# AIR-DISCOVER/TOIST

Measured on AMD Instinct MI355X. Metric: train images/sec/node (640x640, bs=8/GPU) + matcher index bit-match, higher is better.
Workload: dtype bf16; 1 GPU; configs[1]: ResNet-101 + RoBERTa-base + 6+6 transformer, 100 queries, batch 8/GPU 640x640, 16-token captions, detection loss (labels+boxes+cardinality+contrastive_align, 5 aux layers), dropout 0.1, clip 0.1 + AdamW + EMA (fused HIP tail); random-init weights; every step a different batch (4 resident batches, 0..10 targets per image) through fixed-address inputs; global_batch=8, parallelism=dp1, launch=hipGraph replay, decoder=2 XCD-resident launches (toist_xdec_fwd / toist_xdec_bwd, one image per XCD)

## Files before the change

include/toist_hip.h:

```cpp
#ifndef TOIST_HIP_H
#define TOIST_HIP_H

#include <stddef.h>
#include <stdint.h>

#ifdef __cplusplus
extern "C" {
#endif

#define TOIST_OK 0
#define TOIST_EINVAL (-1)
#define TOIST_EHIP (-2)

#define TOIST_ABI_VERSION 1

#if defined(__GNUC__)
#define TOIST_API __attribute__((visibility("default")))
#else
#define TOIST_API
#endif

TOIST_API int toist_version(void);
TOIST_API int toist_last_error(char* buf, size_t cap);

// ... 339 lines not shown
TOIST_API int toist_attn_small_fwd(const void* q, int ldq, const void* kmat, int ldk, const void* v, int ldv, const uint8_t* key_pad, int B, int H, int S,
                         int dh, float scale, float drop_p, uint64_t seed, const uint64_t* seed_dev, void* ctx, int ldo, float* stats,
                         const float* bq, const float* bk, const float* bv, void* stream);
TOIST_API int toist_attn_small_bwd(const void* q, int ldq, const void* kmat, int ldk, const void* v, int ldv, const uint8_t* key_pad, int B, int H, int S,
                         int dh, float scale, float drop_p, uint64_t seed, const uint64_t* seed_dev, const float* stats, const void* dctx,
                         int lddo, void* dq, int lddq, void* dk, int lddk, void* dv, int lddv, const float* bq, const float* bk,
                         const float* bv, void* stream);

TOIST_API int toist_conv3x3_small(int dgrad, const void* src, const void* w, const float* shift, const void* res, void* out, int n_img, int H, int W,
                        int c_src, int c_out, int w_co, int w_ci, void* stream);

TOIST_API int toist_wgrad3x3_small_blocks(void);
TOIST_API int toist_wgrad3x3_small(const void* dy, const void* x, float* ws, int n_img, int H, int W, int c_in, int c_out, void* stream);

TOIST_API int toist_lsap(const float* cost, const int64_t* offset, const int32_t* rows, const int32_t* cols, int ld ,
               int n, int max_rows, int max_cols,
               int64_t max_cells , const int64_t* out_off, int64_t* row_idx, int64_t* col_idx, int32_t* status, void* stream);

#define TOIST_GEMM_DEFER_REDUCE 2
#define TOIST_GEMM_SPLIT_EPILOGUE 4
#define TOIST_GEMM_COLSUM_SLICES 32768
TOIST_API int toist_gemm_pick_tile(const toist_gemm* desc);
typedef struct toist_reduce_desc {
    const float* ws;
    float* out;
    const float* rscale;
    int32_t splits, M, N, ldc;
    float alpha;
    int32_t accumulate;
} toist_reduce_desc;
TOIST_API int toist_gemm_effective_split(const toist_gemm* desc);
TOIST_API int toist_splitk_reduce_batch(const toist_reduce_desc* descs, int n, void* stream);

TOIST_API int toist_opt_chunk_elems(void);
TOIST_API int toist_opt_sqnorm(const toist_opt_tensor* table, const int64_t* grads, const int32_t* chunks, int n_chunks, float* partial, void* stream);
TOIST_API int toist_opt_finish_norm(const float* partial, int n_chunks, float max_norm, float beta1, float beta2, toist_opt_state* state, void* stream);
TOIST_API int toist_opt_finish_norm_guarded(const float* partial, int n_chunks, float max_norm, float beta1, float beta2, toist_opt_state* state,
                        const int32_t* const* veto_i32, int n_veto_i32, const float* const* veto_f32, int n_veto_f32, void* stream);
TOIST_API int toist_opt_adamw_ema(const toist_opt_tensor* table, const int64_t* grads, const int32_t* chunks, int n_chunks,
                        const toist_opt_group* groups, const toist_opt_state* state, float beta1, float beta2, float eps,
                        float ema_decay, void* stream);
TOIST_API int toist_opt_adamw_ema_blocks(const toist_opt_tensor* table, const int64_t* grads, const int32_t* chunks, int n_chunks,
                               const toist_opt_group* groups, const toist_opt_state* state, float beta1, float beta2, float eps,
                               float ema_decay, int max_blocks, void* stream);

TOIST_API int toist_mask_resize_pack(const float* src, int n, int h0, int w0, int max_h, int max_w, int crop_h, int crop_w, int h, int w,
                           float threshold, uint64_t* bits, void* stream);
TOIST_API int toist_mask_resize_pack_batch(const float* src, int batch, int queries, int h0, int w0, int max_h, int max_w, const int64_t* table,
                                 int cap_h, int cap_w, long long capacity_words, float threshold, uint64_t* bits, void* stream);
TOIST_API int toist_mask_pack(const uint8_t* dense, int n, int h, int w, uint64_t* bits, void* stream);
TOIST_API int toist_mask_unpack(const uint64_t* bits, int n, int h, int w, uint8_t* dense, void* stream);
TOIST_API int toist_mask_area(const uint64_t* bits, int n, int h, int w, uint32_t* area, void* stream);
TOIST_API int toist_mask_iou(const uint64_t* dt, int n_dt, const uint64_t* gt, int n_gt, const uint8_t* iscrowd, const uint32_t* area_dt,
                   const uint32_t* area_gt, int h, int w, double* iou, void* stream);
TOIST_API int toist_mask_rle_count(const uint64_t* bits, int n, int h, int w, int32_t* column_transitions, void* stream);
TOIST_API int toist_mask_rle_emit(const uint64_t* bits, int n, int h, int w, const int64_t* column_offset, uint32_t* positions, void* stream);
TOIST_API int toist_mask_rle_counts(const uint32_t* positions, const int64_t* first_position, const int64_t* first_run, int n, int h, int w,
                          uint32_t* counts, void* stream);

TOIST_API int toist_postprocess(const void* pred_logits, int logits_bf16, const void* pred_boxes, int boxes_bf16, const void* pred_isfinal, int isfinal_bf16,
                      const int64_t* orig_sizes, int B, int Q, int C, float* scores, float* boxes, float* scores_refexp, void* stream);

TOIST_API int toist_coco_match(const double* iou, const int64_t* iou_offset, const double* dt_area, const int64_t* dt_offset, const double* gt_area,
                     const uint8_t* gt_ignore, const uint8_t* gt_crowd, const int64_t* gt_offset, int n_images, const double* area_ranges,
                     int n_ranges, const double* iou_thresholds, int n_thresholds, int32_t* dt_match, uint8_t* dt_ignore,
                     uint8_t* gt_range_ignore, uint8_t* gt_taken, void* stream);
// ... 14 lines not shown
```

toist_amd/backbone.py:

```python
import os
from collections import OrderedDict

import torch
from torch import nn

from .knobs import knob
from . import engine, functions
from . import kernels as k
from . import ops
from .misc import NestedTensor
from .position_encoding import build_position_encoding

BF16 = torch.bfloat16
FUSED_STEM = knob("TOIST_FUSED_STEM", True)


_BN_EPOCH = [0]


class FrozenBatchNorm2d(nn.Module):

    def __init__(self, n):
        super().__init__()
        self.register_buffer("weight", torch.ones(n))
# ... 125 lines not shown
    def _program(self, levels, first=1, last=4, stem=True):
        body = self.body
        bn_cache = {}

        def bn(name):
            if name not in bn_cache:
                bn_cache[name] = body.get_submodule(name).scale_shift()
            return bn_cache[name]

        def prog(tape, ps, images):
            x = images.data
            if stem:
                N, C, H, W = x.shape
                s0, t0 = bn("bn1")
                w1 = engine.krsc(ps["conv1.weight"].w)
                if FUSED_STEM and tuple(w1.shape) == (64, 7, 7, 8) and x.dtype == torch.float32:
                    CH, CW = (H - 1) // 2 + 1, (W - 1) // 2 + 1
                    pooled = torch.empty(N, (CH - 1) // 2 + 1, (CW - 1) // 2 + 1, 64, dtype=BF16, device=x.device)
                    k.stem_fwd(x.contiguous(), w1, t0, pooled)
                else:
                    xin = torch.empty(N, H, W, 8, dtype=BF16, device=x.device)
                    k.pack_image(x.contiguous(), xin)
                    y = ops.conv2d(xin, w1, stride=2, pad=3, shift=t0, act=k.ACT_RELU, cin_real=C)
                    OH, OW = (y.shape[1] + 2 - 3) // 2 + 1, (y.shape[2] + 2 - 3) // 2 + 1
                    pooled = torch.empty(N, OH, OW, 64, dtype=BF16, device=x.device)
                    k.maxpool3x3s2(y, pooled)
                    del y
                cur = engine.Var(pooled, needs_grad=False)
            else:
                cur = images
            outs = []
            for li in range(first, last + 1):
                layer = getattr(body, f"layer{li}")
                for bi, blk in enumerate(layer):
                    pre = f"layer{li}.{bi}."
                    Wd = {"conv1": ps[pre + "conv1.weight"], "conv2": ps[pre + "conv2.weight"], "conv3": ps[pre + "conv3.weight"]}
                    bnd = {"bn1": bn(pre + "bn1"), "bn2": bn(pre + "bn2"), "bn3": bn(pre + "bn3")}
                    has_down = blk.downsample is not None
                    if has_down:
                        Wd["down"] = ps[pre + "downsample.0.weight"]
                        bnd["down"] = bn(pre + "downsample.1")
                    train = Wd["conv1"].g is not None
                    nxt = engine.bottleneck(tape, cur, Wd, bnd, blk.stride, has_down, train)
                    nxt.needs_grad = train
                    cur = nxt
                if li in levels:
                    outs.append(cur)
            return outs, None

        return prog

    @staticmethod
    def _with_output_masks(prog, premasked):
        def wrapped(tape, ps, img):
            outs, extra = prog(tape, ps, img)
            finals = []
            for oi, o in enumerate(outs):
                f = engine.Var(o.data, needs_grad=o.needs_grad)

                def bwd(o=o, f=f, oi=oi):
                    g = f.take_grad()
                    if g is None or not o.needs_grad:
                        return
                    gm = g if oi in premasked else torch.where(o.data > 0, g, torch.zeros_like(g))
                    engine.accumulate(o, gm)

                tape.record(bwd)
                finals.append(f)
            return finals, extra
        return wrapped

    STAGES = ((1, 2, True), (3, 3, False), (4, 4, False))

    def forward_native(self, images, levels=(4,), premasked=(), stage_cuts=None):
        if stage_cuts is not None and tuple(levels) == (4,):
            return self._forward_staged(images, premasked, stage_cuts)
        named = engine.named_cache(self, "body", lambda: OrderedDict(self.body.named_parameters()))
        wrapped = self._with_output_masks(self._program(levels), premasked)
        return functions.run_program(wrapped, named, [images], cache=self._cache, training=self.training, transforms=self._transforms(),
                                     group_wgrads=True, store_once=lambda n, t: t.dim() == 4)

    def _forward_staged(self, images, premasked, stage_cuts):
        tr_all = self._transforms()
        caches = self.__dict__.setdefault("_stage_caches", [{} for _ in self.STAGES])
        x = images
        for si, (first, last, stem) in enumerate(self.STAGES):
            def build(first=first, last=last, stem=stem):
                keep = tuple(f"layer{li}." for li in range(first, last + 1)) + (("conv1.",) if stem else ())
                return OrderedDict((n, p) for n, p in self.body.named_parameters() if n.startswith(keep))
            named = engine.named_cache(self, f"body.stage{si}", build)
            tr = {n: f for n, f in tr_all.items() if n in named}
            is_last = si == len(self.STAGES) - 1
            prog = self._program((last,), first, last, stem)
            wrapped = self._with_output_masks(prog, premasked if is_last else (0,))
            (y,) = functions.run_program(wrapped, named, [x], cache=caches[si], training=self.training, transforms=tr, group_wgrads=True,
                                         store_once=lambda n, t: t.dim() == 4)
            if not is_last and y.requires_grad:
                leaf = y.detach().requires_grad_(True)
                stage_cuts.append((f"backbone.layer{last}", y, leaf))
                y = leaf
            x = y
        return (x,)

    def forward(self, tensor_list: NestedTensor):
        levels = (1, 2, 3, 4) if self.return_interm_layers else (4,)
        feats = self.forward_native(tensor_list.tensors, levels)
        out = OrderedDict()
        names = [str(i) for i in range(len(levels))] if self.return_interm_layers else ["0"]
        for name, f in zip(names, feats):
            x = f.permute(0, 3, 1, 2).float()
            mask = nearest_mask(tensor_list.mask, x.shape[-2:])
            out[name] = NestedTensor(x, mask)
        return out


_NEAREST_IDX = {}


# ... 43 lines not shown
```

toist_amd/csrc/gemm.hip:

```cpp
#include <cstdlib>
#include <type_traits>

#include "common.h"
#include "gemm_route.h"

namespace toist {


__device__ __forceinline__ float gelu_f(float v) { return 0.5f * v * (1.f + erff(v * 0.70710678118654752f)); }
__device__ __forceinline__ float gelu_grad_f(float a) {
    return 0.5f * (1.f + erff(a * 0.70710678118654752f)) + a * 0.3989422804014327f * __expf(-0.5f * a * a);
}

template <int N, typename F>
__device__ __forceinline__ void static_for(F&& f) {
    if constexpr (N > 0) {
        static_for<N - 1>(f);
        f(std::integral_constant<int, N - 1>{});
    }
}

struct EpiRow {
    long long crow;
    long long rrow;
// ... 2330 lines not shown
#undef TOIST_PANEL2
#undef TOIST_PANEL2_ONE
    return TOIST_OK;
}

#ifndef GEMM_UNIT
template <int NS>
static int launch_gemm128_ring(const toist_gemm& d, hipStream_t st) {
    static std::atomic<unsigned long long> done{0};
    constexpr int LDS = NS * G8_STAGE_BYTES;
    if (!lds_attr_once_flag(done, [] {
            return hipFuncSetAttribute((const void*)gemm128_kernel<TOIST_A_ROWK, TOIST_B_ROWK, NS>, hipFuncAttributeMaxDynamicSharedMemorySize, LDS) == hipSuccess &&
                   hipFuncSetAttribute((const void*)gemm128_kernel<TOIST_A_ROWK, TOIST_B_KROW, NS>, hipFuncAttributeMaxDynamicSharedMemorySize, LDS) == hipSuccess &&
                   hipFuncSetAttribute((const void*)gemm128_kernel<TOIST_A_CONV, TOIST_B_ROWK, NS>, hipFuncAttributeMaxDynamicSharedMemorySize, LDS) == hipSuccess &&
                   hipFuncSetAttribute((const void*)gemm128_kernel<TOIST_A_CONVT, TOIST_B_KROW, NS>, hipFuncAttributeMaxDynamicSharedMemorySize, LDS) == hipSuccess;
        })) {
        set_last_error("toist_gemm_bf16: cannot enable %d bytes of LDS for the 128x128 kernel", LDS);
        return TOIST_EHIP;
    }
    const int tiles = ((d.M + G8_BM - 1) / G8_BM) * ((d.N + G8_BN - 1) / G8_BN);
    dim3 grid((tiles + 7) & ~7, 1, 1);
    if (d.a_kind == TOIST_A_CONV) hipLaunchKernelGGL((gemm128_kernel<TOIST_A_CONV, TOIST_B_ROWK, NS>), grid, dim3(512), LDS, st, d);
    else if (d.a_kind == TOIST_A_CONVT) hipLaunchKernelGGL((gemm128_kernel<TOIST_A_CONVT, TOIST_B_KROW, NS>), grid, dim3(512), LDS, st, d);
    else if (d.b_kind == TOIST_B_KROW) hipLaunchKernelGGL((gemm128_kernel<TOIST_A_ROWK, TOIST_B_KROW, NS>), grid, dim3(512), LDS, st, d);
    else hipLaunchKernelGGL((gemm128_kernel<TOIST_A_ROWK, TOIST_B_ROWK, NS>), grid, dim3(512), LDS, st, d);
    return TOIST_OK;
}

static int launch_gemm128(const toist_gemm& d, hipStream_t st) {
    static const int ring = (int)tuning_knob("TOIST_G8_RING", 5);
    return (ring == 5 && d.K >= 5 * G8_BK) ? launch_gemm128_ring<5>(d, st) : launch_gemm128_ring<4>(d, st);
}

static int launch_gemm256w(const toist_gemm& d, hipStream_t st) {
    static std::atomic<unsigned long long> done{0};
    if (!lds_attr_once_flag(done, [] {
            return hipFuncSetAttribute((const void*)gemm256w_kernel<TOIST_B_KROW>, hipFuncAttributeMaxDynamicSharedMemorySize, G9_LDS) == hipSuccess &&
                   hipFuncSetAttribute((const void*)gemm256w_kernel<TOIST_B_CONVX>, hipFuncAttributeMaxDynamicSharedMemorySize, G9_LDS) == hipSuccess;
        })) {
        set_last_error("toist_gemm_bf16: cannot enable %d bytes of LDS for the 256x128 weight-gradient kernel", G9_LDS);
        return TOIST_EHIP;
    }
    const toist_gemm& dd = d;
    const int tiles = (d.M / G9_BM) * (d.N / G9_BN);
    const int nz = dd.batch * dd.split_k;
    dim3 grid((tiles + 7) & ~7, nz, 1);
    if (nz >= 8) grid = dim3(8 * ((nz + 7) / 8) * tiles, 1, 1);
    if (d.b_kind == TOIST_B_CONVX) hipLaunchKernelGGL((gemm256w_kernel<TOIST_B_CONVX>), grid, dim3(512), G9_LDS, st, dd);
    else hipLaunchKernelGGL((gemm256w_kernel<TOIST_B_KROW>), grid, dim3(512), G9_LDS, st, dd);
    return TOIST_OK;
}

static int launch_gemm128w(const toist_gemm& d, hipStream_t st) {
    static std::atomic<unsigned long long> done{0};
    if (!lds_attr_once_flag(done, [] {
            return hipFuncSetAttribute((const void*)gemm128w_kernel<TOIST_B_KROW, 4>, hipFuncAttributeMaxDynamicSharedMemorySize, 4 * G8_STAGE_BYTES) == hipSuccess &&
                   hipFuncSetAttribute((const void*)gemm128w_kernel<TOIST_B_CONVX, 4>, hipFuncAttributeMaxDynamicSharedMemorySize, 4 * G8_STAGE_BYTES) == hipSuccess &&
                   hipFuncSetAttribute((const void*)gemm128w_kernel<TOIST_B_KROW, 5>, hipFuncAttributeMaxDynamicSharedMemorySize, 5 * G8_STAGE_BYTES) == hipSuccess &&
                   hipFuncSetAttribute((const void*)gemm128w_kernel<TOIST_B_CONVX, 5>, hipFuncAttributeMaxDynamicSharedMemorySize, 5 * G8_STAGE_BYTES) == hipSuccess;
        })) {
        set_last_error("toist_gemm_bf16: cannot enable %d bytes of LDS for the 128x128 weight-gradient kernel", 5 * G8_STAGE_BYTES);
        return TOIST_EHIP;
    }
    const int tiles = ((d.M + G8_BM - 1) / G8_BM) * ((d.N + G8_BN - 1) / G8_BN);
    const toist_gemm& dd = d;
    const int nz = dd.batch * dd.split_k;
// ... 328 lines not shown
    const gemm_verdict ok = gemm_check(d);
    if (ok.code != TOIST_OK) { set_last_error("%s", ok.msg); return ok.code; }
    const gemm_plan r = gemm_route(d);
    if (r.code != TOIST_OK) { set_last_error("%s", r.msg); return r.code; }
    d.batch = r.batch, d.batch_inner = r.batch_inner, d.split_k = r.split;
    hipStream_t st = (hipStream_t)stream;
    const char* what = "toist_gemm_bf16";
    int rc;
    switch (r.family) {
        case GEMM_128: rc = launch_gemm128(d, st); what = "toist_gemm_bf16(gemm128)"; break;
        case GEMM_CONV3: rc = launch_conv3(d, st); what = "toist_gemm_bf16(conv3)"; break;
        case GEMM_PANEL: rc = r.ring == 1 ? launch_panel(d, st) : launch_panel2(d, r.ring, st); what = "toist_gemm_bf16(panel)"; break;
        case GEMM_128W: rc = launch_gemm128w(d, st); break;
        case GEMM_256W: rc = launch_gemm256w(d, st); break;
        default:
            rc = r.tile == 65 ? launch_tiles_b(r.tile, d, r.ring, st)
               : (r.tile == 130 || r.tile == 134) ? launch_tiles_c(r.tile, d, r.ring, st) : launch_tiles_a(r.tile, d, r.ring, st);
            break;
    }
    if (rc != TOIST_OK) return rc;
    rc = check_launch(what);
    if (rc != TOIST_OK || r.post == GEMM_POST_NONE || r.post == GEMM_POST_DEFERRED) return rc;
    if (r.post == GEMM_POST_EPILOGUE) {
        const long long chunks = (long long)d.M * ((d.N + 7) / 8);
        hipLaunchKernelGGL(splitk_epilogue_kernel, dim3((unsigned)((chunks + 255) / 256)), dim3(256), 0, st, d);
        return check_launch("toist_gemm_bf16(splitk epilogue)");
    }
    const long long total4 = ((long long)d.M * d.N) / 4;
    int grid = (int)((total4 + 255) / 256 > 2048 ? 2048 : (total4 + 255) / 256);
    hipLaunchKernelGGL(splitk_reduce_kernel, dim3(grid), dim3(256), 0, st, (const float*)d.workspace, d.split_k, d.M, d.N, d.epi.alpha,
                       d.epi.rscale, d.epi.accumulate, (float*)d.c, d.ldc);
    return check_launch("toist_gemm_bf16(splitk reduce)");
}
#endif
```

toist_amd/csrc/gemm_route.cpp:

```cpp
#include "gemm_route.h"

#include <cstddef>
#include <cstdio>

#include "tuning.h"

namespace toist {

static bool aligned16(const void* p) { return (((size_t)p) & 15) == 0; }

static void normalise(toist_gemm& d) {
    if (d.batch <= 0) d.batch = 1;
    if (d.batch_inner <= 0) d.batch_inner = 1;
    if (d.split_k <= 0) d.split_k = 1;
}

#define GEMM_REQUIRE(v, cond, ...) \
    do { if ((v).code == TOIST_OK && !(cond)) { (v).code = TOIST_EINVAL; std::snprintf((v).msg, sizeof((v).msg), __VA_ARGS__); } } while (0)

gemm_verdict gemm_check(const toist_gemm& desc) {
    gemm_verdict v{};
    toist_gemm d = desc;
    GEMM_REQUIRE(v, d.M > 0 && d.N > 0 && d.K > 0, "toist_gemm_bf16: bad shape M=%d N=%d K=%d", d.M, d.N, d.K);
    normalise(d);
// ... 238 lines not shown
        GEMM_REQUIRE(r, gemm128_applies(d), "toist_gemm_bf16: the 128x128 kernel does not cover this call");
    } else if (d.tile == 131 || (d.tile == 0 && d.a_kind == TOIST_A_CONVT && conv3_applies(d))) {
        r.family = GEMM_CONV3, r.tile = 131;
        GEMM_REQUIRE(r, conv3_applies(d), "toist_gemm_bf16: the 3x3 halo kernel does not cover this call");
    } else if (code == 135 || (d.tile == 0 && panel_sized && panel_applies(d))) {
        r.family = GEMM_PANEL, r.tile = 135;
        GEMM_REQUIRE(r, panel_applies(d), "toist_gemm_bf16: the short-K panel kernel does not cover this call");
        static const int def_variant = (int)tuning_knob("TOIST_PANEL_VARIANT", 0);
        const int variant = r.ring ? r.ring : def_variant;
        r.ring = (variant == 1 || !panel2_applies(d)) ? 1 : variant == 255 ? 0 : variant;
    } else {
        r.tile = code;
        if (code == 137) GEMM_REQUIRE(r, gemm128w_applies(d), "toist_gemm_bf16: the 128x128 weight-gradient kernel does not cover this call");
        if (code == 138) GEMM_REQUIRE(r, gemm256w_applies(d), "toist_gemm_bf16: the 256x128 weight-gradient kernel does not cover this call");
        if (const int wt = wgrad_tile_replaced(d)) r.tile = wt;
        if (r.tile == 0) r.tile = auto_tile(d);
        r.family = r.tile == 137 ? GEMM_128W : r.tile == 138 ? GEMM_256W : GEMM_TILES;
    }
    r.split = clamp_split(d.split_k, d.K, r.tile);
    r.post = r.split <= 1 ? GEMM_POST_NONE : (d.flags & TOIST_GEMM_DEFER_REDUCE) ? GEMM_POST_DEFERRED
           : (d.flags & TOIST_GEMM_SPLIT_EPILOGUE) ? GEMM_POST_EPILOGUE : GEMM_POST_REDUCE;
    if (r.family == GEMM_TILES || r.family == GEMM_128W || r.family == GEMM_256W) {
        if (d.flags & TOIST_GEMM_COLSUM_SLICES)
            GEMM_REQUIRE(r, r.split > 1, "toist_gemm_bf16: TOIST_GEMM_COLSUM_SLICES with a split that clamps to 1 (see toist_gemm_effective_split)");
        if (d.b_kind == TOIST_B_KROW && d.b.kin > 0) GEMM_REQUIRE(r, (d.b.kin % 8) == 0, "toist_gemm_bf16: kin %% 8 != 0");
    }
    if (r.family == GEMM_TILES) {
        GEMM_REQUIRE(r, generic_tile(r.tile), "toist_gemm_bf16: bad tile code %d", r.tile);
        GEMM_REQUIRE(r, generic_operands(d.a_kind, d.b_kind), "toist_gemm_bf16: unsupported operand kinds a=%d b=%d", d.a_kind, d.b_kind);
    }
    return r;
}

}

extern "C" int toist_gemm_pick_tile(const toist_gemm* desc) { return desc == nullptr ? 0 : toist::gemm_route(*desc).tile; }

extern "C" int toist_gemm_effective_split(const toist_gemm* desc) {
    if (desc == nullptr) return 0;
    toist_gemm d = *desc;
    if (d.workspace == nullptr) d.workspace = (float*)16;
    return toist::gemm_route(d).split;
}
```

toist_amd/csrc/gemm_route.h:

```cpp
#pragma once
#include "../../include/toist_hip.h"

namespace toist {

constexpr int C3_BM = 128, C3_BK = 64, C3_NP = 28;
constexpr int G8_BM = 128, G8_BN = 128, G8_BK = 64;
constexpr int G9_BM = 256, G9_BN = 128, G9_NS = 6;

enum gemm_family {
    GEMM_TILES = 0,
    GEMM_CONV3,
    GEMM_PANEL,
    GEMM_128,
    GEMM_128W,
    GEMM_256W
};

enum gemm_post {
    GEMM_POST_NONE = 0,
    GEMM_POST_REDUCE,
    GEMM_POST_EPILOGUE,
    GEMM_POST_DEFERRED
};

struct gemm_verdict {
    int code;
    char msg[320];
};

struct gemm_plan : gemm_verdict {
    int family;
    int tile;
    int ring;
    int batch, batch_inner, split;
    int post;
};

gemm_verdict gemm_check(const toist_gemm& desc);
gemm_plan gemm_route(const toist_gemm& desc);
bool lean_epilogue_ok(const toist_gemm& d);

}
```

toist_amd/engine.py:

```python
import math

import weakref

import torch

from . import kernels as k
from . import ops
from .knobs import knob

BF16 = torch.bfloat16


class Var:

    __slots__ = ("data", "grad", "needs_grad", "drop", "gdrop", "plus", "raw_grad")

    def __init__(self, data, needs_grad=True):
        self.data = data
        self.grad = None
        self.needs_grad = needs_grad
        self.raw_grad = False
        self.plus = None
        self.drop = None
        self.gdrop = None
# ... 749 lines not shown

def text_attention_block(tape, x, proj, Wpacked, Wo, bo, key_pad, B, L, H):
    D = Wo.w.shape[0]
    dh = D // H
    M = B * L
    dev = x.data.device
    p = tape.drop_p
    scale = 1.0 / math.sqrt(dh)
    qkv = ops.linear(x.data, Wpacked)
    seed_p = tape.next_seed() if p > 0 else 0
    ctx = torch.empty(M, D, dtype=BF16, device=dev)
    stats = torch.empty(B * H, L, 2, dtype=torch.float32, device=dev)
    bias = [b.f32 for _, b in proj]
    k.attn_small_fwd(qkv[:, :D], qkv[:, D:2 * D], qkv[:, 2 * D:], key_pad, B, H, L, dh, scale, p, seed_p, ctx, stats, *bias)
    out, head = _out_proj(tape, ctx, Wo, bo, x, p)

    def bwd():
        dctx = head()
        if dctx is None:
            return
        dqkv = torch.empty(M, 3 * D, dtype=BF16, device=dev)
        k.attn_small_bwd(qkv[:, :D], qkv[:, D:2 * D], qkv[:, 2 * D:], key_pad, B, H, L, dh, scale, p, seed_p, stats, dctx,
                         dqkv[:, :D], dqkv[:, D:2 * D], dqkv[:, 2 * D:], *bias)
        for i, (W, b) in enumerate(proj):
            if W.g is not None:
                tape.linear_wgrad(dqkv[:, i * D:(i + 1) * D], x.data, W, b)
        if x.needs_grad:
            x.grad = ops.linear_dgrad(dqkv, Wpacked, res=x.grad)

    tape.record(bwd)
    return out


def bottleneck(tape, x, W, bn, stride, has_down, train):
    w1, w2, w3 = krsc(W["conv1"].w), krsc(W["conv2"].w), krsc(W["conv3"].w)
    s1, t1 = bn["bn1"]
    s2, t2 = bn["bn2"]
    s3, t3 = bn["bn3"]
    a1 = ops.conv2d(x.data, w1, shift=t1, act=k.ACT_RELU)
    a2 = ops.conv2d(a1, w2, stride=stride, pad=1, shift=t2, act=k.ACT_RELU)
    if has_down:
        wd = krsc(W["down"].w)
        sd, td = bn["down"]
        idn = ops.conv2d(x.data, wd, stride=stride, shift=td)
    else:
        idn = x.data
    y = ops.conv2d(a2, w3, shift=t3, res=idn, act=k.ACT_RELU)
    if has_down:
        del idn
    out = Var(y)
    if not train:
        return out
    H, Wd = x.data.shape[1], x.data.shape[2]

    def bwd():
        g3 = out.take_grad()
        if g3 is None:
            return
        tape.conv_wgrad(g3, a2, w3.shape, krsc(W["conv3"].g), s3, view=W["conv3"])
        g2 = ops.conv2d_dgrad(g3, w3, a2.shape[1:3], act=k.ACT_MASK_POS, aux=a2)
        tape.conv_wgrad(g2, a1, w2.shape, krsc(W["conv2"].g), s2, stride=stride, pad=1, view=W["conv2"])
        g1 = ops.conv2d_dgrad(g2, w2, (H, Wd), stride=stride, pad=1, act=k.ACT_MASK_POS, aux=a1)
        tape.conv_wgrad(g1, x.data, w1.shape, krsc(W["conv1"].g), s1, view=W["conv1"])
        if has_down:
            tape.conv_wgrad(g3, x.data, wd.shape, krsc(W["down"].g), sd, stride=stride, view=W["down"])
        if not x.needs_grad:
            return
        prev = x.take_grad()
        if has_down:
            if stride == 1:
                gx = ops.conv2d_dgrad(g3, wd, (H, Wd), res=prev)
            else:
                gx = prev if prev is not None else torch.zeros_like(x.data)
                ops.conv2d_dgrad(g3, wd, (H, Wd), stride=stride, out=gx, res=gx if prev is not None else None)
        else:
            gx = g3
            if prev is not None:
                k.add(prev, g3, prev)
                gx = prev
        x.grad = ops.conv2d_dgrad(g1, w1, (H, Wd), res=gx, act=k.ACT_MASK_POS, aux=x.data)

    tape.record(bwd)
    return out
```

toist_amd/kernels.py:

```python
import ctypes
import os

import torch

from . import _lib
from .folds import FOLDS, _raw_stream
from .knobs import knob
from ._lib import (A_CONV, A_CONVT, A_KROW, A_ROWK, ACT_GELU, ACT_GELU_BWD, ACT_MASK_POS, ACT_NONE, ACT_RELU,
                   ACT_SIGMOID, ACT_SIGMOID_BWD, B_CONVX, B_KROW, B_ROWK, Epilogue, Gemm, Operand)

__all__ = [
    "A_ROWK", "A_KROW", "A_CONV", "A_CONVT", "B_ROWK", "B_KROW", "B_CONVX", "ACT_NONE", "ACT_RELU", "ACT_GELU",
    "ACT_SIGMOID", "ACT_MASK_POS", "ACT_GELU_BWD", "ACT_SIGMOID_BWD", "ConvGeom", "operand", "gemm", "matcher",
    "layernorm_fwd", "layernorm_bwd", "softmax_fwd", "softmax_bwd", "colsum", "add", "dropout", "pack_image", "maxpool3x3s2", "stem_fwd",
    "unpack_nhwc", "sine_position", "embed_fwd", "embed_bwd", "criterion_fwd", "criterion_bwd", "attnmap_softmax_fwd", "attnmap_softmax_bwd",
    "groupnorm_fwd", "groupnorm_apply", "groupnorm_bwd", "upsample_add", "upsample_add_bwd", "sum_queries", "sum_segments", "upsample_add_rows", "mask_stage_fwd", "mask_loss_fwd", "mask_loss_bwd",
]


PROFILE = None
SEED_DEV = None
FORCE_TILE = 0
FORCE_SPLIT = 0
DEBUG_FLAGS = 0
# ... 198 lines not shown
            d.flags |= GEMM_COLSUM_SLICES
            folds.insert(0, dict(ws=cs.data_ptr(), out=a_colsum, splits=eff, M=1, N=M, ldc=M, keep=(cs,),
                                 now=not d.flags & GEMM_DEFER_REDUCE, when_busy="now"))
    if DEBUG_WS is not None and split_k <= 1:
        d.workspace = _p(DEBUG_WS, torch.float32)
        d.flags |= 2048 | DEBUG_FLAGS
    prof, events = PROFILE, None
    if prof is not None:
        if not flops:
            flops = 2 * M * N * K * max(batch, 1)
        t = int(_lib.lib().toist_gemm_pick_tile(ctypes.byref(d)))
        key = (t, a_kind, b_kind)
        want = prof["key"]
        if want is not None and not (want(key) if callable(want) else (key == want or (isinstance(want, (set, frozenset)) and key in want))):
            prof["other"][key] = prof["other"].get(key, 0) + flops
        else:
            events = torch.cuda.Event(enable_timing=True), torch.cuda.Event(enable_timing=True)
            events[0].record()
    _lib.check(_lib.lib().toist_gemm_bf16(ctypes.byref(d), _stream()), "toist_gemm_bf16")
    if events is not None:
        events[1].record()
    for f in folds:
        FOLDS.queue(**f)
    if events is None:
        return
    ta = max(int(a.R) * int(a.S), 1) if a_kind in (A_CONV, A_CONVT) else 1
    tb = max(int(b.R) * int(b.S), 1) if b_kind == B_CONVX else 1
    nb = max(batch, 1)
    nbytes = 2 * M * K * nb // ta + 2 * N * K * nb // tb + (4 if c.dtype == torch.float32 else 2) * M * N * nb
    nbytes += 2 * M * N * nb * ((res is not None) + (aux is not None) + (pre_out is not None))
    prof["records"].append((*events, flops, key, (M, N, K, nb, split_k, ta * tb), nbytes))


def matcher(logits, boxes, tgt_boxes, pos_map, tgt_off, match_off, max_T, w_class, w_bbox, w_giou, src_idx, tgt_idx,
            status, cost_out=None):
    L, B, Q, K = logits.shape
    _lib.check(
        _lib.lib().toist_matcher(_p(logits, torch.float32), _p(boxes, torch.float32), _p(tgt_boxes, torch.float32),
                                 _p(pos_map, torch.float32), _p(tgt_off, torch.int32), _p(match_off, torch.int32), L, B, Q,
                                 K, max_T, w_class, w_bbox, w_giou, _p(src_idx, torch.int64), _p(tgt_idx, torch.int64),
                                 _p(status, torch.int32), _p(cost_out, torch.float32), _stream()), "toist_matcher")


def layernorm_fwd(x, gamma, beta, eps, y, mean=None, rstd=None, add=None, y2=None):
    rows, D = x.shape
    _lib.check(
        _lib.lib().toist_layernorm_fwd(_p(x, torch.bfloat16), _p(gamma, torch.float32), _p(beta, torch.float32), eps, rows, D,
                                       _p(y, torch.bfloat16), _p(mean, torch.float32), _p(rstd, torch.float32), _p(add, torch.bfloat16),
                                       _p(y2, torch.bfloat16), _stream()),
        "toist_layernorm_fwd")


LN_DEFER = knob("TOIST_LN_DEFER", True)


def _queue_ln_param_grads(blocks, D, dgamma, dbeta):
    partials = FOLDS.acquire(2 * blocks * D, dgamma.device, (dgamma, dbeta))
    for i, out in enumerate((dgamma, dbeta)):
        FOLDS.queue(partials.data_ptr() + 4 * i * blocks * D, out, blocks, 1, D, D)
    return partials


def layernorm_bwd(dy, x, mean, rstd, gamma, dx, dgamma=None, dbeta=None, dx_drop=None, drop_p=0.0, seed=0, defer=False):
    rows, D = x.shape
    partials, blocks = None, 0
    if defer and LN_DEFER and dgamma is not None:
# ... 654 lines not shown
```

Measured before the change: 705.2 images/s.

## Fuse conv3 and next block's conv1 across layer3 bottlenecks in one kernel

Adds a conv_pair HIP kernel that computes a bottleneck's conv3 (with residual, shift and ReLU) and immediately feeds the tile from LDS into the next block's conv1 GEMM, writing both outputs. It also fuses the backward pair: the next block's conv1 dgrad and the current block's conv3 dgrad, with masked-ReLU epilogues. The result is stashed for reuse. It applies only to layer3 blocks with C=256, stride 1 and no downsample. The goal is to avoid re-reading the 1024-wide activation from HBM and to save kernel launches. In exchange it adds a large, hand-scheduled kernel with fixed wait counts and inline asm, plus cross-block state passing that is fragile.

```diff
diff --git a/include/toist_hip.h b/include/toist_hip.h
--- a/include/toist_hip.h
+++ b/include/toist_hip.h
@@ -395,6 +395,24 @@
 TOIST_API int toist_gemm_effective_split(const toist_gemm* desc);
 TOIST_API int toist_splitk_reduce_batch(const toist_reduce_desc* descs, int n, void* stream);
 
+typedef struct toist_conv_pair {
+    int32_t M, C;
+    int32_t dgrad;
+    int32_t lda;
+    const void* a;
+    const void* w_first;
+    const void* w_second;
+    const float* shift_mid;
+    const float* shift_out;
+    const void* res;
+    const void* aux_mid;
+    const void* aux_out;
+    void* mid;
+    void* out;
+    int32_t ldr, ldaux_mid, ldaux_out, ldmid, ldout, reserved;
+} toist_conv_pair;
+TOIST_API int toist_conv_pair_bf16(const toist_conv_pair* desc, void* stream);
+
 TOIST_API int toist_opt_chunk_elems(void);
 TOIST_API int toist_opt_sqnorm(const toist_opt_tensor* table, const int64_t* grads, const int32_t* chunks, int n_chunks, float* partial, void* stream);
 TOIST_API int toist_opt_finish_norm(const float* partial, int n_chunks, float max_norm, float beta1, float beta2, toist_opt_state* state, void* stream);
diff --git a/toist_amd/backbone.py b/toist_amd/backbone.py
--- a/toist_amd/backbone.py
+++ b/toist_amd/backbone.py
@@ -181,6 +181,7 @@
             outs = []
             for li in range(first, last + 1):
                 layer = getattr(body, f"layer{li}")
+                take = None
                 for bi, blk in enumerate(layer):
                     pre = f"layer{li}.{bi}."
                     Wd = {"conv1": ps[pre + "conv1.weight"], "conv2": ps[pre + "conv2.weight"], "conv3": ps[pre + "conv3.weight"]}
@@ -190,7 +191,15 @@
                         Wd["down"] = ps[pre + "downsample.0.weight"]
                         bnd["down"] = bn(pre + "downsample.1")
                     train = Wd["conv1"].g is not None
-                    nxt = engine.bottleneck(tape, cur, Wd, bnd, blk.stride, has_down, train)
+                    give = None
+                    if k.CONV_PAIR and li == 3 and bi + 1 < len(layer):
+                        nb = layer[bi + 1]
+                        if nb.stride == 1 and nb.downsample is None and tuple(nb.conv1.weight.shape[:2]) == (256, 1024) \
+                                and tuple(blk.conv3.weight.shape[:2]) == (1024, 256):
+                            npre = f"layer{li}.{bi + 1}."
+                            give = engine.pair_link(ps[npre + "conv1.weight"], bn(npre + "bn1")[1])
+                    nxt = engine.bottleneck(tape, cur, Wd, bnd, blk.stride, has_down, train, take=take, give=give)
+                    take = give
                     nxt.needs_grad = train
                     cur = nxt
                 if li in levels:
@@ -233,6 +242,7 @@
         tr_all = self._transforms()
         caches = self.__dict__.setdefault("_stage_caches", [{} for _ in self.STAGES])
         x = images
+        assert sum(first <= 3 <= last for first, last, _ in self.STAGES) == 1
         for si, (first, last, stem) in enumerate(self.STAGES):
             def build(first=first, last=last, stem=stem):
                 keep = tuple(f"layer{li}." for li in range(first, last + 1)) + (("conv1.",) if stem else ())
diff --git a/toist_amd/csrc/gemm.hip b/toist_amd/csrc/gemm.hip
--- a/toist_amd/csrc/gemm.hip
+++ b/toist_amd/csrc/gemm.hip
@@ -2386,6 +2386,285 @@
     return (ring == 5 && d.K >= 5 * G8_BK) ? launch_gemm128_ring<5>(d, st) : launch_gemm128_ring<4>(d, st);
 }
 
+__device__ __forceinline__ u32x4_t load16_asm(const i32x4_t& r, const int byte_off) {
+    u32x4_t v;
+    asm volatile("buffer_load_dwordx4 %0, %1, %2, 0 offen" : "=&v"(v) : "v"(byte_off), "s"(r) : "memory");
+    return v;
+}
+__device__ __forceinline__ u32x2_t load8_asm(const i32x4_t& r, const int byte_off) {
+    u32x2_t v;
+    asm volatile("buffer_load_dwordx2 %0, %1, %2, 0 offen" : "=&v"(v) : "v"(byte_off), "s"(r) : "memory");
+    return v;
+}
+
+constexpr int CP_TILE_BYTES = 128 * 64 * 2;
+constexpr int CP_STEP_BYTES = 2 * CP_TILE_BYTES;
+constexpr int CP_NS = 3;
+constexpr int CP_STEPS = 32;
+constexpr int CP_A_OFF = 0;
+constexpr int CP_MID_OFF = CP_A_OFF + CP_BM * CP_C * 2;
+constexpr int CP_RING_OFF = CP_MID_OFF + CP_BM * 128 * 2;
+constexpr int CP_SHIFT_OFF = CP_RING_OFF + CP_NS * CP_STEP_BYTES;
+constexpr int CP_LDS = CP_SHIFT_OFF + 5 * CP_C * 4;
+static_assert(CP_LDS <= 160 * 1024, "conv_pair_kernel: LDS");
+
+template <bool DG, bool SPLIT>
+__global__ __launch_bounds__(512, 2) void conv_pair_kernel(const toist_conv_pair p, const float alpha) {
+    constexpr int BK = 64, KT = BK * CP_BM;
+    constexpr int C = CP_C, C4 = 4 * CP_C;
+    extern __shared__ __attribute__((aligned(16))) unsigned char lds_raw[];
+    bf16_t* const smem = reinterpret_cast<bf16_t*>(lds_raw);
+    const int tid = threadIdx.x, lane = tid & 63, wave = __builtin_amdgcn_readfirstlane(tid >> 6);
+    const int g = lane >> 4, c16 = lane & 15;
+    const int wm1 = wave >> 2, wn1 = wave & 3;
+    const int M = p.M;
+    const int nt = (M + CP_BM - 1) / CP_BM, per = (nt + 7) >> 3;
+    const int tile_m = (int)(blockIdx.x & 7) * per + (int)(blockIdx.x >> 3);
+    if (tile_m >= nt) return;
+    const int m0 = tile_m * CP_BM;
+    const unsigned lds0 = (unsigned)(size_t)lds_raw;
+    const unsigned ring0 = lds0 + CP_RING_OFF;
+
+    float* const sh = reinterpret_cast<float*>(lds_raw + CP_SHIFT_OFF);
+    sh[tid] = (!DG && p.shift_mid) ? p.shift_mid[tid] : 0.f;
+    sh[tid + 512] = (!DG && p.shift_mid) ? p.shift_mid[tid + 512] : 0.f;
+    if (tid < C) sh[C4 + tid] = (!DG && p.shift_out) ? p.shift_out[tid] : 0.f;
+
+    const i32x4_t rsA = make_rsrc(p.a), rsW1 = make_rsrc(p.w_first), rsW2 = make_rsrc(p.w_second), rsMid = make_rsrc(p.mid);
+    const i32x4_t rsR = make_rsrc(p.res), rsXm = make_rsrc(DG ? p.aux_mid : p.res), rsXo = make_rsrc(DG ? p.aux_out : p.res);
+    constexpr int NR = DG ? 4 : 2;
+    auto pcol = [](const int j, const int q) { return 8 * (q >> 2) + 4 * j + (q & 3); };
+
+    int v1[2], v2[2];
+#pragma unroll
+    for (int it = 0; it < 2; ++it) {
+        const int pch = (it * 8 + wave) * 64 + lane;
+        if (DG) {
+            const int krow = pch >> 4, rc = swz_m<128>(krow, pch & 15);
+            v1[it] = (krow * C4 + rc * 8) * 2;
+            v2[it] = (krow * C + rc * 8) * 2;
+        } else {
+            const int row = pch >> 3, kc = swz_k<BK>(row, pch & 7);
+            const int prow = (row & ~31) + pcol((row >> 4) & 1, row & 15);
+            v1[it] = (prow * C + kc * 8) * 2;
+            v2[it] = (row * C4 + kc * 8) * 2;
+        }
+    }
+    auto issue = [&](const int s, const int slot) {
+        const int c = s >> 2, q = s & 3;
+        const unsigned dst = ring0 + (unsigned)(slot * CP_STEP_BYTES) + (unsigned)wave * 1024u;
+#pragma unroll
+        for (int tt = 0; tt < 2; ++tt) {
+            const unsigned d0 = dst + (unsigned)(tt * CP_TILE_BYTES);
+            if (q < 2) {
+                const int so = DG ? ((2 * q + tt) * BK * C4 + 128 * c) * 2 : (128 * c * C + (2 * q + tt) * BK) * 2;
+                dma16s(d0, rsW1, v1[0], so);
+                dma16s(d0 + 8192u, rsW1, v1[1], so);
+            } else {
+                const int k0 = 128 * c + BK * (q - 2);
+                const int so = DG ? (k0 * C + 128 * tt) * 2 : (128 * tt * C4 + k0) * 2;
+                dma16s(d0, rsW2, v2[0], so);
+                dma16s(d0 + 8192u, rsW2, v2[1], so);
+            }
+        }
+    };
+
+    asm volatile("s_waitcnt vmcnt(0)" ::: "memory");
+    {
+        const int pa = wave * 64 + lane, ar = pa >> 3, akc = swz_k<BK>(ar, pa & 7);
+        const int va = (m0 + ar < M) ? ((m0 + ar) * p.lda + akc * 8) * 2 : OOB;
+#pragma unroll
+        for (int it = 0; it < 4; ++it) dma16s(lds0 + (unsigned)(CP_A_OFF + it * KT * 2) + (unsigned)wave * 1024u, rsA, va, it * BK * 2);
+    }
+    issue(0, 0);
+    issue(1, 1);
+
+    f32x4_t acc1[2][2];
+    f32x4_t acc2[SPLIT ? 2 : 1][4][2];
+#pragma unroll
+    for (int h = 0; h < (SPLIT ? 2 : 1); ++h)
+#pragma unroll
+        for (int i = 0; i < 4; ++i)
+#pragma unroll
+            for (int j = 0; j < 2; ++j) acc2[h][i][j] = f32x4_t{0.f, 0.f, 0.f, 0.f};
+    u32x4_t rres[2], raux[2];
+    const u32x4_t zero4 = {0u, 0u, 0u, 0u};
+    rres[0] = rres[1] = raux[0] = raux[1] = zero4;
+
+    int slot = 0;
+    u32x2_t xo[4][2];
+    auto step_top = [&](const int s, auto qc) {
+        constexpr int q = decltype(qc)::value;
+        if (q == 3 && s + 1 == CP_STEPS) wait_vm<(DG ? 10 : 2)>();
+        else wait_vm<(q == 0 ? 4 : q == 1 ? 4 + NR : q == 2 ? NR + 6 : 6)>();
+        lds_barrier();
+    };
+    auto refill = [&](const int s) {
+        if (s + 2 < CP_STEPS) issue(s + 2, slot >= 1 ? slot - 1 : CP_NS - 1);
+    };
+    auto next_slot = [&]() { slot = slot == CP_NS - 1 ? 0 : slot + 1; };
+
+#pragma unroll 1
+    for (int c = 0; c < 8; ++c) {
+        const int ncol = 128 * c + wn1 * 32 + g * 8;
+        static_for<2>([&](auto uc) {
+            constexpr int u = decltype(uc)::value;
+            const int s = c * 4 + u;
+            step_top(s, uc);
+            refill(s);
+            if (u == 0) {
+#pragma unroll
+                for (int i = 0; i < 2; ++i) {
+#pragma unroll
+                    for (int j = 0; j < 2; ++j) acc1[i][j] = f32x4_t{0.f, 0.f, 0.f, 0.f};
+                    const int m = m0 + wm1 * 32 + i * 16 + c16;
+                    rres[i] = load16_asm(rsR, m < M ? (m * p.ldr + ncol) * 2 : OOB);
+                    if (DG) raux[i] = load16_asm(rsXm, m < M ? (m * p.ldaux_mid + ncol) * 2 : OOB);
+                }
+            }
+            const unsigned char* const sB = lds_raw + CP_RING_OFF + slot * CP_STEP_BYTES;
+#pragma unroll
+            for (int tt = 0; tt < 2; ++tt) {
+                const bf16_t* const sA = smem + CP_A_OFF / 2 + (2 * u + tt) * KT;
+                const bf16_t* const sBt = reinterpret_cast<const bf16_t*>(sB + tt * CP_TILE_BYTES);
+#pragma unroll
+                for (int ks = 0; ks < 2; ++ks) {
+                    bf16x8_t af[2], bfr[2];
+#pragma unroll
+                    for (int i = 0; i < 2; ++i) af[i] = fragment<false, CP_BM, BK>(sA, wm1 * 32 + i * 16, ks, g, c16);
+#pragma unroll
+                    for (int j = 0; j < 2; ++j)
+                        bfr[j] = DG ? fragment_perm8<128, BK>(sBt, wn1 * 32, j, ks, g, c16) : fragment<false, 128, BK>(sBt, wn1 * 32 + j * 16, ks, g, c16);
+#pragma unroll
+                    for (int i = 0; i < 2; ++i)
+#pragma unroll
+                        for (int j = 0; j < 2; ++j) acc1[i][j] = __builtin_amdgcn_mfma_f32_16x16x32_bf16(bfr[j], af[i], acc1[i][j], 0, 0, 0);
+                }
+            }
+            next_slot();
+        });
+        {
+            if (DG) asm volatile("s_waitcnt vmcnt(4)" : "+v"(rres[0]), "+v"(rres[1]), "+v"(raux[0]), "+v"(raux[1]) : : "memory");
+            else asm volatile("s_waitcnt vmcnt(4)" : "+v"(rres[0]), "+v"(rres[1]) : : "memory");
+            float csh[8];
+            const f32x4_t s0 = *reinterpret_cast<const f32x4_t*>(sh + ncol), s1 = *reinterpret_cast<const f32x4_t*>(sh + ncol + 4);
+#pragma unroll
+            for (int e = 0; e < 4; ++e) { csh[e] = s0[e]; csh[4 + e] = s1[e]; }
+#pragma unroll
+            for (int i = 0; i < 2; ++i) {
+                const int r = wm1 * 32 + i * 16 + c16, m = m0 + r;
+                float v[8];
+#pragma unroll
+                for (int jj = 0; jj < 2; ++jj)
+#pragma unroll
+                    for (int e = 0; e < 4; ++e) v[jj * 4 + e] = acc1[i][jj][e] * alpha + csh[jj * 4 + e];
+                add8(v, rres[i]);
+                if (DG) {
+                    const u32x4_t x4 = raux[i];
+                    v[0] = __uint_as_float(x4[0] << 16) > 0.f ? v[0] : 0.f; v[1] = __uint_as_float(x4[0] & 0xffff0000u) > 0.f ? v[1] : 0.f;
+                    v[2] = __uint_as_float(x4[1] << 16) > 0.f ? v[2] : 0.f; v[3] = __uint_as_float(x4[1] & 0xffff0000u) > 0.f ? v[3] : 0.f;
+                    v[4] = __uint_as_float(x4[2] << 16) > 0.f ? v[4] : 0.f; v[5] = __uint_as_float(x4[2] & 0xffff0000u) > 0.f ? v[5] : 0.f;
+                    v[6] = __uint_as_float(x4[3] << 16) > 0.f ? v[6] : 0.f; v[7] = __uint_as_float(x4[3] & 0xffff0000u) > 0.f ? v[7] : 0.f;
+                }
+                u32x4_t o = {pack2bf(v[0], v[1]), pack2bf(v[2], v[3]), pack2bf(v[4], v[5]), pack2bf(v[6], v[7])};
+                if (!DG) {
+                    unsigned r0, r1, r2, r3;
+                    asm("v_pk_max_i16 %0, %1, 0" : "=v"(r0) : "v"(o[0]));
+                    asm("v_pk_max_i16 %0, %1, 0" : "=v"(r1) : "v"(o[1]));
+                    asm("v_pk_max_i16 %0, %1, 0" : "=v"(r2) : "v"(o[2]));
+                    asm("v_pk_max_i16 %0, %1, 0" : "=v"(r3) : "v"(o[3]));
+                    o[0] = r0; o[1] = r1; o[2] = r2; o[3] = r3;
+                }
+                const int cb = wn1 * 32 + g * 8;
+                *reinterpret_cast<u32x4_t*>(lds_raw + CP_MID_OFF + (cb >> 6) * KT * 2 + (r * BK + swz_k<BK>(r, (cb & 63) >> 3) * 8) * 2) = o;
+                store16_asm(rsMid, m < M ? (m * p.ldmid + ncol) * 2 : OOB, o);
+            }
+        }
+        static_for<2>([&](auto ktc) {
+            constexpr int kt = decltype(ktc)::value;
+            const int s = c * 4 + 2 + kt;
+            step_top(s, std::integral_constant<int, 2 + kt>{});
+            refill(s);
+            if (DG && s == CP_STEPS - 2) {
+#pragma unroll
+                for (int i = 0; i < 4; ++i)
+#pragma unroll
+                    for (int j = 0; j < 2; ++j) {
+                        const int m = m0 + i * 16 + c16;
+                        xo[i][j] = load8_asm(rsXo, m < M ? (m * p.ldaux_out + wave * 32 + j * 16 + g * 4) * 2 : OOB);
+                    }
+            }
+            const bf16_t* const sM = smem + CP_MID_OFF / 2 + kt * KT;
+            const bf16_t* const sBh = reinterpret_cast<const bf16_t*>(lds_raw + CP_RING_OFF + slot * CP_STEP_BYTES + (wave >> 2) * CP_TILE_BYTES);
+#pragma unroll
+            for (int ks = 0; ks < 2; ++ks) {
+                bf16x8_t af[4], bfr[2];
+#pragma unroll
+                for (int i = 0; i < 4; ++i) af[i] = fragment<false, CP_BM, BK>(sM, i * 16, ks, g, c16);
+#pragma unroll
+                for (int j = 0; j < 2; ++j) bfr[j] = fragment<DG, 128, BK>(sBh, (wave & 3) * 32 + j * 16, ks, g, c16);
+#pragma unroll
+                for (int i = 0; i < 4; ++i)
+#pragma unroll
+                    for (int j = 0; j < 2; ++j)
+                        acc2[SPLIT ? ks : 0][i][j] = __builtin_amdgcn_mfma_f32_16x16x32_bf16(bfr[j], af[i], acc2[SPLIT ? ks : 0][i][j], 0, 0, 0);
+            }
+            next_slot();
+        });
+    }
+    if (DG) {
+#pragma unroll
+        for (int i = 0; i < 4; ++i) asm volatile("s_waitcnt vmcnt(0)" : "+v"(xo[i][0]), "+v"(xo[i][1]) : : "memory");
+    } else {
+        wait_vm<0>();
+    }
+
+    bf16_t* const outp = (bf16_t*)p.out;
+#pragma unroll
+    for (int i = 0; i < 4; ++i) {
+        const int m = m0 + i * 16 + c16;
+#pragma unroll
+        for (int j = 0; j < 2; ++j) {
+            const int col = wave * 32 + j * 16 + g * 4;
+            f32x4_t a = acc2[0][i][j];
+            if (SPLIT) a = a + acc2[SPLIT ? 1 : 0][i][j];
+            const f32x4_t sv = *reinterpret_cast<const f32x4_t*>(sh + C4 + col);
+            float v[4];
+#pragma unroll
+            for (int e = 0; e < 4; ++e) v[e] = a[e] * alpha + sv[e];
+            if (m < M) {
+                if (DG) {
+                    const u32x2_t x2 = xo[i][j];
+                    v[0] = __uint_as_float(x2[0] << 16) > 0.f ? v[0] : 0.f; v[1] = __uint_as_float(x2[0] & 0xffff0000u) > 0.f ? v[1] : 0.f;
+                    v[2] = __uint_as_float(x2[1] << 16) > 0.f ? v[2] : 0.f; v[3] = __uint_as_float(x2[1] & 0xffff0000u) > 0.f ? v[3] : 0.f;
+                } else {
+#pragma unroll
+                    for (int e = 0; e < 4; ++e) v[e] = fmaxf(v[e], 0.f);
+                }
+                *reinterpret_cast<uint2*>(outp + (size_t)m * p.ldout + col) = make_uint2(pack2bf(v[0], v[1]), pack2bf(v[2], v[3]));
+            }
+        }
+    }
+}
+
+static int launch_conv_pair(const toist_conv_pair& d, const bool split, hipStream_t st) {
+    const int nt = (d.M + CP_BM - 1) / CP_BM, per = (nt + 7) / 8;
+    const dim3 grid(8u * (unsigned)per, 1, 1);
+#define TOIST_CONV_PAIR(DG, SP)                                                                                                            \
+    do {                                                                                                                                   \
+        static std::atomic<unsigned long long> done{0};                                                                                    \
+        if (!lds_attr_once_flag(done, [] { return hipFuncSetAttribute((const void*)conv_pair_kernel<DG, SP>, hipFuncAttributeMaxDynamicSharedMemorySize, CP_LDS) == hipSuccess; })) { \
+            set_last_error("toist_conv_pair_bf16: cannot enable %d bytes of LDS", CP_LDS);                                                 \
+            return TOIST_EHIP;                                                                                                             \
+        }                                                                                                                                  \
+        hipLaunchKernelGGL((conv_pair_kernel<DG, SP>), grid, dim3(512), CP_LDS, st, d, 1.f);                                               \
+    } while (0)
+    if (d.dgrad) { if (split) TOIST_CONV_PAIR(true, true); else TOIST_CONV_PAIR(true, false); }
+    else { if (split) TOIST_CONV_PAIR(false, true); else TOIST_CONV_PAIR(false, false); }
+#undef TOIST_CONV_PAIR
+    return TOIST_OK;
+}
+
 static int launch_gemm256w(const toist_gemm& d, hipStream_t st) {
     static std::atomic<unsigned long long> done{0};
     if (!lds_attr_once_flag(done, [] {
@@ -2780,4 +3059,15 @@
                        d.epi.rscale, d.epi.accumulate, (float*)d.c, d.ldc);
     return check_launch("toist_gemm_bf16(splitk reduce)");
 }
+
+extern "C" int toist_conv_pair_bf16(const toist_conv_pair* desc, void* stream) {
+    using namespace toist;
+    TOIST_REQUIRE(desc != nullptr, "toist_conv_pair_bf16: null descriptor");
+    const toist_conv_pair d = *desc;
+    const gemm_verdict ok = pair_check(d);
+    if (ok.code != TOIST_OK) { set_last_error("%s", ok.msg); return ok.code; }
+    const bool split = gemm_route(pair_second_gemm(d)).family == GEMM_128;
+    const int rc = launch_conv_pair(d, split, (hipStream_t)stream);
+    return rc != TOIST_OK ? rc : check_launch("toist_conv_pair_bf16");
+}
 #endif
diff --git a/toist_amd/csrc/gemm_route.cpp b/toist_amd/csrc/gemm_route.cpp
--- a/toist_amd/csrc/gemm_route.cpp
+++ b/toist_amd/csrc/gemm_route.cpp
@@ -294,6 +294,53 @@
     return r;
 }
 
+gemm_verdict pair_check(const toist_conv_pair& d) {
+    gemm_verdict v{};
+    const long long lim = 1ll << 30;
+    GEMM_REQUIRE(v, d.M > 0 && d.C == CP_C, "toist_conv_pair_bf16: bad shape M=%d C=%d (C = %d only)", d.M, d.C, CP_C);
+    GEMM_REQUIRE(v, d.dgrad == 0 || d.dgrad == 1, "toist_conv_pair_bf16: dgrad = %d (0 or 1)", d.dgrad);
+    GEMM_REQUIRE(v, d.a && d.w_first && d.w_second && d.mid && d.out, "toist_conv_pair_bf16: null operand");
+    GEMM_REQUIRE(v, d.res != nullptr, "toist_conv_pair_bf16: res is required");
+    if (d.dgrad) {
+        GEMM_REQUIRE(v, d.aux_mid && d.aux_out, "toist_conv_pair_bf16: the data gradient needs aux_mid and aux_out");
+        GEMM_REQUIRE(v, !d.shift_mid && !d.shift_out, "toist_conv_pair_bf16: the data gradient takes no shift");
+    } else {
+        GEMM_REQUIRE(v, !d.aux_mid && !d.aux_out, "toist_conv_pair_bf16: aux_mid / aux_out belong to the data gradient (dgrad = 1)");
+    }
+    GEMM_REQUIRE(v, aligned16(d.a) && aligned16(d.w_first) && aligned16(d.w_second) && aligned16(d.res) && aligned16(d.mid) && aligned16(d.out) &&
+                        aligned16(d.aux_mid) && aligned16(d.aux_out) && aligned16(d.shift_mid) && aligned16(d.shift_out),
+                 "toist_conv_pair_bf16: every pointer must be 16-byte aligned");
+    const int C = CP_C, C4 = 4 * CP_C;
+    GEMM_REQUIRE(v, d.lda >= C && d.ldout >= C && d.ldmid >= C4 && d.ldr >= C4 && (d.lda % 8) == 0 && (d.ldout % 8) == 0 && (d.ldmid % 8) == 0 && (d.ldr % 8) == 0,
+                 "toist_conv_pair_bf16: leading dimensions must cover the row and be multiples of 8 (lda=%d ldmid=%d ldr=%d ldout=%d)", d.lda, d.ldmid,
+                 d.ldr, d.ldout);
+    if (d.dgrad)
+        GEMM_REQUIRE(v, d.ldaux_mid >= C4 && d.ldaux_out >= C && (d.ldaux_mid % 8) == 0 && (d.ldaux_out % 8) == 0,
+                     "toist_conv_pair_bf16: leading dimensions must cover the row and be multiples of 8 (ldaux_mid=%d ldaux_out=%d)", d.ldaux_mid, d.ldaux_out);
+    const long long rows = (long long)((d.M + CP_BM - 1) / CP_BM) * CP_BM;
+    GEMM_REQUIRE(v, rows * d.lda < lim && rows * d.ldmid < lim && rows * d.ldr < lim && rows * d.ldout < lim &&
+                        (!d.dgrad || (rows * d.ldaux_mid < lim && rows * d.ldaux_out < lim)),
+                 "toist_conv_pair_bf16: M = %d rows exceed the 2 GiB byte offsets of the kernel", d.M);
+    return v;
+}
+
+bool pair_applies(const toist_conv_pair& desc) { return pair_check(desc).code == TOIST_OK; }
+
+toist_gemm pair_second_gemm(const toist_conv_pair& p) {
+    toist_gemm d{};
+    d.M = p.M, d.N = p.C, d.K = 4 * p.C;
+    d.a_kind = TOIST_A_ROWK, d.b_kind = p.dgrad ? TOIST_B_KROW : TOIST_B_ROWK;
+    d.a.ptr = p.mid, d.a.ld = p.ldmid;
+    d.b.ptr = p.w_second, d.b.ld = p.dgrad ? p.C : 4 * p.C;
+    d.c = p.out, d.ldc = p.ldout;
+    d.batch = d.batch_inner = d.split_k = 1;
+    d.epi.alpha = 1.f;
+    d.epi.shift = p.shift_out;
+    d.epi.act = p.dgrad ? TOIST_ACT_MASK_POS : TOIST_ACT_RELU;
+    d.epi.aux = p.aux_out, d.epi.ldaux = p.dgrad ? p.ldaux_out : 0;
+    return d;
+}
+
 }
 
 extern "C" int toist_gemm_pick_tile(const toist_gemm* desc) { return desc == nullptr ? 0 : toist::gemm_route(*desc).tile; }
diff --git a/toist_amd/csrc/gemm_route.h b/toist_amd/csrc/gemm_route.h
--- a/toist_amd/csrc/gemm_route.h
+++ b/toist_amd/csrc/gemm_route.h
@@ -40,4 +40,9 @@
 gemm_plan gemm_route(const toist_gemm& desc);
 bool lean_epilogue_ok(const toist_gemm& d);
 
+constexpr int CP_BM = 64, CP_C = 256;
+gemm_verdict pair_check(const toist_conv_pair& desc);
+bool pair_applies(const toist_conv_pair& desc);
+toist_gemm pair_second_gemm(const toist_conv_pair& desc);
+
 }
diff --git a/toist_amd/engine.py b/toist_amd/engine.py
--- a/toist_amd/engine.py
+++ b/toist_amd/engine.py
@@ -805,12 +805,24 @@
     return out
 
 
-def bottleneck(tape, x, W, bn, stride, has_down, train):
+def pair_link(w1_next, t1_next):
+    return {"w1": w1_next, "t1": t1_next}
+
+
+def _pair_shapes_ok(a2, w3, w1n, idn):
+    C = a2.shape[-1]
+    return C == 256 and tuple(w3.shape) == (4 * C, 1, 1, C) and tuple(w1n.shape) == (C, 1, 1, 4 * C) and idn.is_contiguous() \
+        and tuple(idn.shape) == (*a2.shape[:3], 4 * C) and a2.is_contiguous()
+
+
+def bottleneck(tape, x, W, bn, stride, has_down, train, take=None, give=None):
     w1, w2, w3 = krsc(W["conv1"].w), krsc(W["conv2"].w), krsc(W["conv3"].w)
     s1, t1 = bn["bn1"]
     s2, t2 = bn["bn2"]
     s3, t3 = bn["bn3"]
-    a1 = ops.conv2d(x.data, w1, shift=t1, act=k.ACT_RELU)
+    a1 = take.pop("a1", None) if take is not None else None
+    if a1 is None:
+        a1 = ops.conv2d(x.data, w1, shift=t1, act=k.ACT_RELU)
     a2 = ops.conv2d(a1, w2, stride=stride, pad=1, shift=t2, act=k.ACT_RELU)
     if has_down:
         wd = krsc(W["down"].w)
@@ -818,7 +830,18 @@
         idn = ops.conv2d(x.data, wd, stride=stride, shift=td)
     else:
         idn = x.data
-    y = ops.conv2d(a2, w3, shift=t3, res=idn, act=k.ACT_RELU)
+    w1n = krsc(give["w1"].w) if give is not None else None
+    if give is not None and (k.CONV_PAIR & 1) and _pair_shapes_ok(a2, w3, w1n, idn):
+        C, M = a2.shape[-1], a2.numel() // a2.shape[-1]
+        y = torch.empty(*a2.shape[:3], 4 * C, dtype=BF16, device=a2.device)
+        a1n = torch.empty_like(a2)
+        k.conv_pair(a2.view(M, C), w3.view(4 * C, C), w1n.view(C, 4 * C), idn.view(M, 4 * C), y.view(M, 4 * C), a1n.view(M, C),
+                    shift_mid=t3, shift_out=give["t1"])
+        give["a1"] = a1n
+    else:
+        y = ops.conv2d(a2, w3, shift=t3, res=idn, act=k.ACT_RELU)
+    if give is not None and train and (k.CONV_PAIR & 2) and _pair_shapes_ok(a2, w3, w1n, y):
+        give["w3"], give["a2"] = w3, a2
     if has_down:
         del idn
     out = Var(y)
@@ -828,10 +851,14 @@
 
     def bwd():
         g3 = out.take_grad()
+        stash = give.pop("g", None) if give is not None else None
         if g3 is None:
             return
         tape.conv_wgrad(g3, a2, w3.shape, krsc(W["conv3"].g), s3, view=W["conv3"])
-        g2 = ops.conv2d_dgrad(g3, w3, a2.shape[1:3], act=k.ACT_MASK_POS, aux=a2)
+        if stash is not None and stash[0] is g3:
+            g2 = stash[1]
+        else:
+            g2 = ops.conv2d_dgrad(g3, w3, a2.shape[1:3], act=k.ACT_MASK_POS, aux=a2)
         tape.conv_wgrad(g2, a1, w2.shape, krsc(W["conv2"].g), s2, stride=stride, pad=1, view=W["conv2"])
         g1 = ops.conv2d_dgrad(g2, w2, (H, Wd), stride=stride, pad=1, act=k.ACT_MASK_POS, aux=a1)
         tape.conv_wgrad(g1, x.data, w1.shape, krsc(W["conv1"].g), s1, view=W["conv1"])
@@ -840,6 +867,15 @@
         if not x.needs_grad:
             return
         prev = x.take_grad()
+        if take is not None and "a2" in take and not has_down and prev is None and stride == 1 and g3.is_contiguous():
+            C, M = g1.shape[-1], g1.numel() // g1.shape[-1]
+            pa2 = take.pop("a2")
+            gx, g2p = torch.empty_like(x.data), torch.empty_like(pa2)
+            k.conv_pair(g1.view(M, C), w1.view(C, 4 * C), take.pop("w3").view(4 * C, C), g3.view(M, 4 * C), gx.view(M, 4 * C), g2p.view(M, C),
+                        dgrad=True, aux_mid=x.data.view(M, 4 * C), aux_out=pa2.view(M, C))
+            x.grad = gx
+            take["g"] = (gx, g2p)
+            return
         if has_down:
             if stride == 1:
                 gx = ops.conv2d_dgrad(g3, wd, (H, Wd), res=prev)
diff --git a/toist_amd/kernels.py b/toist_amd/kernels.py
--- a/toist_amd/kernels.py
+++ b/toist_amd/kernels.py
@@ -254,6 +254,38 @@
     prof["records"].append((*events, flops, key, (M, N, K, nb, split_k, ta * tb), nbytes))
 
 
+class ConvPair(ctypes.Structure):
+    _fields_ = [("M", ctypes.c_int32), ("C", ctypes.c_int32), ("dgrad", ctypes.c_int32), ("lda", ctypes.c_int32)] + \
+               [(n, ctypes.c_void_p) for n in ("a", "w_first", "w_second", "shift_mid", "shift_out", "res", "aux_mid", "aux_out", "mid", "out")] + \
+               [(n, ctypes.c_int32) for n in ("ldr", "ldaux_mid", "ldaux_out", "ldmid", "ldout", "reserved")]
+
+
+CONV_PAIR = knob("TOIST_CONV_PAIR", 3)
+CONV_PAIR_CALLS = [0, 0]
+
+
+def conv_pair(a, w_first, w_second, res, mid, out, *, dgrad=False, shift_mid=None, shift_out=None, aux_mid=None, aux_out=None):
+    M, C = a.shape
+    for t in (a, res, mid, out, aux_mid, aux_out):
+        if t is not None and (t.dim() != 2 or t.stride(1) != 1 or t.shape[0] != M):
+            raise ValueError("conv_pair: operands are [M, width] views with contiguous rows")
+    if tuple(w_first.shape) != ((C, 4 * C) if dgrad else (4 * C, C)) or tuple(w_second.shape) != ((4 * C, C) if dgrad else (C, 4 * C)) \
+            or not (w_first.is_contiguous() and w_second.is_contiguous()):
+        raise ValueError("conv_pair: weights are contiguous [4C, C] / [C, 4C] (forward) or [C, 4C] / [4C, C] (data gradient)")
+    if tuple(res.shape) != (M, 4 * C) or tuple(mid.shape) != (M, 4 * C) or tuple(out.shape) != (M, C):
+        raise ValueError("conv_pair: res / mid are [M, 4C], out is [M, C]")
+    d = ConvPair()
+    d.M, d.C, d.dgrad, d.lda = M, C, 1 if dgrad else 0, a.stride(0)
+    d.a, d.w_first, d.w_second = _p(a, torch.bfloat16), _p(w_first, torch.bfloat16), _p(w_second, torch.bfloat16)
+    d.shift_mid, d.shift_out = _p(shift_mid, torch.float32), _p(shift_out, torch.float32)
+    d.res, d.ldr = _p(res, torch.bfloat16), res.stride(0)
+    d.aux_mid, d.ldaux_mid = _p(aux_mid, torch.bfloat16), aux_mid.stride(0) if aux_mid is not None else 0
+    d.aux_out, d.ldaux_out = _p(aux_out, torch.bfloat16), aux_out.stride(0) if aux_out is not None else 0
+    d.mid, d.ldmid, d.out, d.ldout = _p(mid, torch.bfloat16), mid.stride(0), _p(out, torch.bfloat16), out.stride(0)
+    CONV_PAIR_CALLS[1 if dgrad else 0] += 1
+    _lib.check(_lib.lib().toist_conv_pair_bf16(ctypes.cast(ctypes.pointer(d), ctypes.c_void_p), _stream()), "toist_conv_pair_bf16")
+
+
 def matcher(logits, boxes, tgt_boxes, pos_map, tgt_off, match_off, max_T, w_class, w_bbox, w_giou, src_idx, tgt_idx,
             status, cost_out=None):
     L, B, Q, K = logits.shape
```

New measurement: 715.3 images/s (median of 6 runs). +1.4%, better.
